# klepo/k-Wave-Fluid-CUDA

Measured on AMD Instinct MI355X. Metric: time-steps/sec on 256^3 heterogeneous grid; achieved HBM GB/s vs roofline, higher is better.
Workload: dtype f32; 1 GPU; 256^3 heterogeneous (c0,rho0,BonA,alpha_coeff arrays), power-law absorption + nonlinear, p0 source, p_raw+p_max on one xy plane (65536 points); fused_kernels=True, fft=hand-written fused FFT passes (kw_fused.hip), device=gfx950:sramecc+:xnack-

## Files before the change

### include/kwave_hip.h

```cpp
#ifndef KWAVE_HIP_H
#define KWAVE_HIP_H

#include <stddef.h>
#include <stdint.h>

#ifdef __cplusplus
extern "C" {
#endif

#define KW_API __attribute__((visibility("default")))

typedef struct kw_ctx kw_ctx;

typedef enum kw_status
{
  KW_OK            = 0,
  KW_ERR_INVALID   = 1,
  KW_ERR_HIP       = 2,
  KW_ERR_FFT       = 3,
  KW_ERR_ALLOC     = 4,
  KW_ERR_STATE     = 5,
  KW_ERR_NO_DEVICE = 6,
  KW_ERR_COMM      = 7
} kw_status;
// ... 39 lines not shown
  uint64_t l2_bytes;
} kw_device_info;

KW_API kw_status   kw_init(int device_id, kw_ctx** out_ctx);
KW_API kw_status   kw_destroy(kw_ctx* ctx);
KW_API const char* kw_last_error(void);
KW_API kw_status   kw_device_info_get(kw_ctx* ctx, kw_device_info* out);
KW_API kw_status   kw_set_stream(kw_ctx* ctx, void* hip_stream);
KW_API void*       kw_get_stream(kw_ctx* ctx);
KW_API kw_status   kw_sync(kw_ctx* ctx);
typedef struct kw_tuning
{
  uint32_t struct_bytes;
  int32_t  side_array;
  int32_t  tail_chunks;
  int32_t  split512;
  int32_t  slab_pipeline;
  int32_t  slab_chunks;
  int32_t  slab_batch;
  int32_t  p2p_blocks_per_peer;
  float    p2p_timeout_s;
  int32_t  plane_kernels;
  uint64_t offgrid_scratch_bytes;
} kw_tuning;
KW_API kw_status   kw_get_tuning(kw_ctx* ctx, kw_tuning* out);
KW_API kw_status   kw_set_tuning(kw_ctx* ctx, const kw_tuning* tuning);
typedef struct kw_graph kw_graph;
KW_API kw_status   kw_graph_begin(kw_ctx* ctx);
KW_API kw_status   kw_graph_end(kw_ctx* ctx, kw_graph** out);
KW_API kw_status   kw_graph_launch(kw_ctx* ctx, kw_graph* g);
KW_API kw_status   kw_graph_destroy(kw_ctx* ctx, kw_graph* g);
KW_API kw_status   kw_measure_copy_bandwidth(kw_ctx* ctx, size_t bytes, int reps, double* out_gbs);
KW_API kw_status   kw_event_create(kw_ctx* ctx, void** out_event);
KW_API kw_status   kw_event_record(kw_ctx* ctx, void* event);
KW_API kw_status   kw_event_synchronize(kw_ctx* ctx, void* event);
KW_API kw_status   kw_event_elapsed_ms(kw_ctx* ctx, void* start, void* stop, float* out_ms);
KW_API kw_status   kw_event_destroy(kw_ctx* ctx, void* event);

typedef struct kw_profile_entry
{
  char     name[64];
  uint64_t calls;
  double   total_ms;
} kw_profile_entry;
KW_API kw_status kw_profile_enable(kw_ctx* ctx, int on);
KW_API int       kw_profile_enabled(kw_ctx* ctx);
// ... 108 lines not shown
KW_API kw_status kw_comm_init_with(kw_ctx* ctx, const char* rccl_library, uint32_t nranks, uint32_t rank, const void* unique_id);
#define KW_COMM_P2P_BLOB_BYTES 1024
KW_API kw_status kw_comm_init_p2p(kw_ctx* ctx, uint32_t nranks, uint32_t rank);
KW_API kw_status kw_comm_p2p_export(kw_ctx* ctx, void* blob, size_t bytes);
KW_API kw_status kw_comm_p2p_connect(kw_ctx* ctx, const void* all_blobs);
KW_API kw_status kw_comm_p2p_emulate(kw_ctx* ctx, float link_gbs, float latency_us);
KW_API kw_status kw_comm_transport(kw_ctx* ctx, int* out_transport);
typedef int (*kw_exchange_fn)(void* user, void* send, void* recv, size_t bytes_per_peer);
KW_API kw_status kw_fused_set_slab(kw_ctx* ctx, uint32_t nranks, uint32_t rank, uint32_t nz_global,
                                   kw_exchange_fn exchange, void* user);
typedef int (*kw_exchange_start_fn)(void* user, void* send, void* recv, size_t bytes_per_peer, int slot);
typedef int (*kw_exchange_wait_fn)(void* user, int slot);
KW_API kw_status kw_fused_set_slab_async(kw_ctx* ctx, kw_exchange_start_fn start, kw_exchange_wait_fn wait);
typedef int (*kw_exchange_piece_fn)(void* user, void* send, void* recv, size_t stride_bytes, size_t offset_bytes, size_t bytes,
                                    int slot);
KW_API kw_status kw_fused_set_slab_pieces(kw_ctx* ctx, kw_exchange_piece_fn start, kw_exchange_wait_fn wait);
KW_API kw_status kw_fused_scratch_bytes(kw_ctx* ctx, size_t* out_bytes_per_array);
KW_API kw_status kw_fused_create_with_scratch(kw_ctx* ctx, void* const s[3], void* const t[3]);
KW_API kw_status kw_fused_supported(kw_ctx* ctx, int* out_supported);
KW_API kw_status kw_fused_create(kw_ctx* ctx);
KW_API kw_status kw_fused_destroy(kw_ctx* ctx);
KW_API kw_status kw_fused_reduced_elems(kw_ctx* ctx, size_t* out_floats);
KW_API kw_status kw_fused_import_reduced(kw_ctx* ctx, float* dst_padded, const float* src_reduced);
KW_API kw_status kw_fused_velocity(kw_ctx* ctx, const float* p, float* ux_sgx, float* uy_sgy, float* uz_sgz,
                                   const float* dt_rho0_sgx, const float* dt_rho0_sgy, const float* dt_rho0_sgz,
                                   const float* pml_x_sgx, const float* pml_y_sgy, const float* pml_z_sgz,
                                   const float* kappa_padded, const float* ddx_k_shift_pos,
                                   const float* ddy_k_shift_pos, const float* ddz_k_shift_pos, int chain_u_spectra);
#define KW_FUSED_CHAIN_U       1
#define KW_FUSED_P_IN_SCRATCH  2
#define KW_FUSED_U_IN_SCRATCH 1
#define KW_FUSED_CHAIN_TERMS  2
KW_API kw_status kw_fused_initial_velocity(kw_ctx* ctx, const float* p, float* ux_sgx, float* uy_sgy, float* uz_sgz,
                                           const float* dt_rho0_sgx, const float* dt_rho0_sgy,
                                           const float* dt_rho0_sgz, const float* kappa_padded,
                                           const float* ddx_k_shift_pos, const float* ddy_k_shift_pos,
                                           const float* ddz_k_shift_pos);
KW_API kw_status kw_fused_density(kw_ctx* ctx, int nonlinear, const float* ux_sgx, const float* uy_sgy,
                                  const float* uz_sgz, float* rho_x, float* rho_y, float* rho_z, const float* pml_x,
                                  const float* pml_y, const float* pml_z, const float* rho0,
                                  const float* kappa_padded, const float* ddx_k_shift_neg,
                                  const float* ddy_k_shift_neg, const float* ddz_k_shift_neg, float* duxdx,
                                  float* duydy, float* duzdz, int terms, const float* b_on_a, float* t0, float* t1,
                                  float* t2, int flags);
KW_API kw_status kw_fused_velocity_gradient(kw_ctx* ctx, const float* ux_sgx, const float* uy_sgy, const float* uz_sgz,
                                            float* duxdx, float* duydy, float* duzdz, const float* kappa_padded,
// ... 112 lines not shown
```

### k-wave-fluid-cuda_amd/capi.py

```python
from __future__ import annotations

import ctypes as C
import os
import re
from typing import Dict, Iterable, Optional

import numpy as np

PKG = os.path.dirname(os.path.abspath(__file__))
ROOT = os.path.dirname(PKG)
LIB_PATH = os.path.join(PKG, "lib", "libkwave_hip.so")
HEADER_PATH = os.path.join(ROOT, "include", "kwave_hip.h")

OP_NONE, OP_RMS, OP_MAX, OP_MIN = 0, 1, 2, 3
SRC_DIRICHLET, SRC_ADDITIVE_NO_CORRECTION, SRC_ADDITIVE = 0, 1, 2


class KWaveError(RuntimeError):
    """Non-zero kw_status; message = kw_last_error() (the reference throws std::runtime_error)."""


class Constants(C.Structure):
    _fields_ = [(n, C.c_uint32) for n in ("nx", "ny", "nz", "n_elements", "nx_complex", "ny_complex", "nz_complex",
                                          "n_elements_complex")] + \
# ... 102 lines not shown
    "kw_comm_init": [_P, C.c_uint32, C.c_uint32, _P],
    "kw_comm_destroy": [_P],
    "kw_comm_info": [_P, C.POINTER(C.c_uint32), C.POINTER(C.c_uint32), C.POINTER(C.c_uint64)],
    "kw_comm_unique_id_from": [C.c_char_p, _P, C.c_size_t],
    "kw_comm_init_with": [_P, C.c_char_p, C.c_uint32, C.c_uint32, _P],
    "kw_comm_init_p2p": [_P, C.c_uint32, C.c_uint32],
    "kw_comm_p2p_export": [_P, _P, C.c_size_t],
    "kw_comm_p2p_connect": [_P, _P],
    "kw_comm_p2p_emulate": [_P, C.c_float, C.c_float],
    "kw_comm_transport": [_P, C.POINTER(C.c_int)],
    "kw_get_tuning": [_P, _P],
    "kw_set_tuning": [_P, _P],
    "kw_fused_set_slab": [_P, C.c_uint32, C.c_uint32, C.c_uint32, _P, _P],
    "kw_fused_set_slab_async": [_P, _P, _P],
    "kw_fused_set_slab_pieces": [_P, _P, _P],
    "kw_fused_scratch_bytes": [_P, C.POINTER(C.c_size_t)],
    "kw_fused_create_with_scratch": [_P, _P, _P],
    "kw_fused_supported": [_P, C.POINTER(C.c_int)],
    "kw_fused_shift_velocity": [_P, C.c_int, _P, _P, _P],
    "kw_fused_create": [_P],
    "kw_fused_destroy": [_P],
    "kw_fused_reduced_elems": [_P, C.POINTER(C.c_size_t)],
    "kw_fused_import_reduced": [_P, _P, _P],
    "kw_fused_velocity": [_P] + [_P] * 14 + [C.c_int],
    "kw_fused_initial_velocity": [_P] + [_P] * 11,
    "kw_fused_density": [_P, C.c_int] + [_P] * 14 + [_P] * 3 + [C.c_int, _P, _P, _P, _P, C.c_int],
    "kw_fused_velocity_gradient": [_P] + [_P] * 10 + [C.c_int],
    "kw_fused_absorption_pressure": [_P] + [_P] * 9 + [C.c_int],
    "kw_fused_absorption_pressure_one": [_P] + [_P] * 6 + [C.c_int, C.c_int],
    "kw_fused_scale_source": [_P, _P, _P],
    "kw_fused_probe": [_P, C.c_int, _P],
    "kw_sample_index": [_P, C.c_int, _P, _P, _P, _U64],
    "kw_sample_index_multi": [_P, C.c_int, _P, _P, _P, _P, C.c_uint64],
    "kw_sample_cuboid": [_P, C.c_int, _P, _P, _P, _P, _P, _U64],
    "kw_sample_all": [_P, C.c_int, _P, _P, _U64],
    "kw_post_processing_rms": [_P, _P, C.c_float, _U64],
    "kw_sample_index_compress": [_P, _P, _P, _P, _P, _U64, C.c_uint32, _P, _P, C.c_uint32, C.c_uint32, C.c_int],
    "kw_sample_index_compress_40b": [_P, _P, _P, _P, _P, _U64, C.c_uint32, _P, _P, C.c_uint32, C.c_uint32, C.c_int, C.c_int, C.c_int],
    "kw_intensity_avg_c_accumulate_40b": [_P, _P, _P, _P, _U64, C.c_uint32, C.c_int, C.c_int],
    "kw_intensity_avg_c_accumulate": [_P, _P, _P, _P, _U64, C.c_uint32],
    "kw_time_shift_series": [_P, _P, _P, _U64, _U64],
    "kw_intensity_avg": [_P, _P, _P, _P, _U64, _U64],
    "kw_q_term_sum": [_P, _P, _P, _P, _P, _U64],
    "kw_divide": [_P, _P, C.c_float, _U64],
    "kw_element_source_row": [_P, _P, _P, _P, _P, C.c_uint32, C.c_uint32, _U64],
    "kw_sample_elements": [_P, _P, _P, _P, _P, C.c_uint32, _U64, _P, C.c_uint32, _P],
# ... 177 lines not shown
                                 C.byref(h)))
    try:
        n_el, nnz = _U64(), _U64()
        check(dev.L.kw_offgrid_size(dev.ctx, h, C.byref(n_el), C.byref(nnz)))
        ptr = np.empty(n_el.value + 1, dtype=np.uint64)
        index = np.empty(nnz.value, dtype=np.uint64)
        weight = np.empty(nnz.value, dtype=np.float32)
        check(dev.L.kw_offgrid_ptr(dev.ctx, h, ptr.ctypes.data))
        check(dev.L.kw_offgrid_entries(dev.ctx, h, index.ctypes.data, weight.ctypes.data))
    finally:
        dev.L.kw_offgrid_free(dev.ctx, h)
    return ptr, index, weight


COMM_ID_BYTES = 128
COMM_P2P_BLOB_BYTES = 1024
TRANSPORTS = {-1: "none", 0: "rccl", 1: "p2p (not connected)", 2: "p2p", 3: "p2p link model"}


class Tuning(C.Structure):
    _fields_ = [("struct_bytes", C.c_uint32), ("side_array", C.c_int32), ("tail_chunks", C.c_int32), ("split512", C.c_int32),
                ("slab_pipeline", C.c_int32), ("slab_chunks", C.c_int32), ("slab_batch", C.c_int32),
                ("p2p_blocks_per_peer", C.c_int32), ("p2p_timeout_s", C.c_float), ("plane_kernels", C.c_int32),
                ("offgrid_scratch_bytes", C.c_uint64)]


def default_tuning() -> Tuning:
    return Tuning(C.sizeof(Tuning), 1, 0, 1, 1, 1, -1, 4, 20.0, 1, 256 << 20)


def make_tuning(spec=None) -> Tuning:
    t = default_tuning()
    for src in (os.environ.get("KW_TUNING"), spec):
        if not src:
            continue
        items = src.items() if isinstance(src, dict) else (kv.split("=", 1) for kv in str(src).replace(" ", ",").split(",") if kv)
        for k, v in items:
            if k not in dict(Tuning._fields_) or k == "struct_bytes":
                raise KWaveError(f"unknown tuning parameter {k!r}")
            setattr(t, k, float(v) if k == "p2p_timeout_s" else int(v))
    return t


def comm_unique_id(rccl_library=None) -> bytes:
    buf = C.create_string_buffer(COMM_ID_BYTES)
    lib = rccl_library.encode() if rccl_library else None
    check(load().kw_comm_unique_id_from(lib, buf, COMM_ID_BYTES))
    return buf.raw


def comm_transport(ctx) -> str:
# ... 10 lines not shown
```

### k-wave-fluid-cuda_amd/csrc/kw_cw.hip

```cpp
#include "kw_fused.hip"

namespace {

template<int L> __global__ __launch_bounds__((Geo<L, nl_z(L)>::THREADS)) void k_zfused_pair(ZArgs a)
{
  using G = Geo<L, nl_z(L)>;
  constexpr int R1 = G::R1, R2 = G::R2;
  constexpr bool WA = (R2 == G::TPL) || ((G::NL * R2) % 64 == 0 && 64 % G::NL == 0);
  __shared__ float2 lds[G::LDSB];
  __shared__ float2 twl[G::TWN];
  load_twiddles<L>(twl, a.tw);
  const int       c     = threadIdx.x % G::NL;
  const int       j     = threadIdx.x / G::NL;
  const TileCoord tc    = tile_coord<G::NL>(a.nxc, a.P, a.side_off, gridDim.y, c);
  if (tc.dead) return;
  const uint32_t ky     = tc.pos;
  const bool     valid  = tc.valid;
  const uint32_t zstr   = a.ny * tc.pitch;
  const uint32_t base   = ky * tc.pitch + (tc.side ? 0u : tc.kx) + tc.off;
  const uint32_t basel  = ky * tc.pitch + tc.col + tc.off;
  constexpr int  OPV    = op_vec(R2);
  const uint32_t opbase = tc.side ? a.op_side_off + (((ky / NLMAX) * (R2 / OPV) * R1 + j) * NLMAX + ky % NLMAX) * OPV
                                  : (((ky * (a.Pop / NLMAX) + tc.col / NLMAX) * (R2 / OPV) * R1 + j) * NLMAX + tc.col % NLMAX) * OPV;
  const float2* __restrict__ in0 = a.in[0];
  const float2* __restrict__ in1 = a.in[1];

  float2 v[R1];
  if (ACTW(R2, j))
  {
    const uint32_t lb = (basel + static_cast<uint32_t>(j) * zstr) * static_cast<uint32_t>(sizeof(float2));
#pragma unroll
    for (int n1 = 0; n1 < R1; n1++) v[n1] = ld_uni<WA>(in0, static_cast<uint64_t>(n1 * R2) * zstr, lb);
  }
  float gr[R2], gi[R2];
  if (ACTW(R1, j))
  {
    load_op_run<R2, R1>(gr, a.op[0], opbase);
    load_op_run<R2, R1>(gi, a.op[1], opbase);
  }
  lds_barrier();

  if (ACTW(R2, j))
  {
    step_a<L, kFwd>(v, j, twl);
#pragma unroll
    for (int k1 = 0; k1 < R1; k1++) lds[k1 * G::SF + j * G::NL + c] = v[k1];
    uint32_t lb = basel + static_cast<uint32_t>(j) * zstr;
    asm volatile("" : "+v"(lb));
#pragma unroll
    for (int n1 = 0; n1 < R1; n1++)
      v[n1] = ld_uni<WA>(in1, static_cast<uint64_t>(n1 * R2) * zstr, lb * static_cast<uint32_t>(sizeof(float2)));
  }
  lds_barrier();
  float2 X[R2], Y[R2];
  if (ACTW(R1, j))
  {
#pragma unroll
    for (int n2 = 0; n2 < R2; n2++) X[n2] = lds[j * G::SF + n2 * G::NL + c];
    Dft<R2, kFwd>::run(X);
  }
  lds_barrier();
  if (ACTW(R2, j))
  {
    step_a<L, kFwd>(v, j, twl);
#pragma unroll
    for (int k1 = 0; k1 < R1; k1++) lds[k1 * G::SF + j * G::NL + c] = v[k1];
  }
  lds_barrier();
  if (ACTW(R1, j))
  {
#pragma unroll
    for (int n2 = 0; n2 < R2; n2++) Y[n2] = lds[j * G::SF + n2 * G::NL + c];
    Dft<R2, kFwd>::run(Y);
#pragma unroll
    for (int k2 = 0; k2 < R2; k2++)
    {
      const float2 x = X[k2], y = Y[k2];
      X[k2] = make_float2(gr[k2] * x.x - gi[k2] * y.x, gr[k2] * x.y - gi[k2] * y.y);
      Y[k2] = make_float2(gi[k2] * x.x + gr[k2] * y.x, gi[k2] * x.y + gr[k2] * y.y);
    }
  }

  float2 r[R1];
  inverse_from_regs<L, false, G::NL>(X, r, lds, c, j, twl);
  if (ACTW(R2, j) && valid)
  {
    float2* __restrict__ out = a.out[0];
    uint32_t ob = base + static_cast<uint32_t>(j) * zstr;
    asm volatile("" : "+v"(ob));
#pragma unroll
    for (int q2 = 0; q2 < R1; q2++) st_uni<WA>(out, static_cast<uint64_t>(R2 * q2) * zstr, ob * static_cast<uint32_t>(sizeof(float2)), r[q2]);
  }
  lds_barrier();
  inverse_from_regs<L, false, G::NL>(Y, r, lds, c, j, twl);
  if (ACTW(R2, j) && valid)
  {
// ... 331 lines not shown
      CV<V>::store(g.phase + s, vp);
    }
  }
}

}

namespace kwfused {

kw_status zfused_pair(kw_ctx* ctx, ZArgs a)
{
  const auto& f = ctx->fused;
  KW_PROF(ctx, "k_zfused_pair");
  a.tw          = f.tw[2];
  a.divider     = 1.0f;
  a.nxc         = f.nxm;
  a.side_off    = f.side_off;
  a.op_side_off = f.side_off;
  a.P           = f.P;
  a.Pop         = f.P;
  a.ny          = f.nyl;
  a.nz          = f.nz_global;
  a.narr        = 2;
  const uint32_t side_tile = (f.side_off != 0) ? 1u : 0u;
  if (f.nz_global == 512 && f.split512)
  {
    LAUNCH((k_zfused_pair_split<512>), dim3(f.P / NLMAX + side_tile, f.nyl, 1), dim3(Geo<256>::THREADS), a);
    return KW_OK;
  }
  const dim3 grid(z_tiles(f.P, f.nz_global) + side_tile, f.nyl, 1);
#define M(LEN) LAUNCH((k_zfused_pair<LEN>), grid, dim3((Geo<LEN, nl_z(LEN)>::THREADS)), a)
  KW_LEN_SWITCH(f.nz_global, M)
#undef M
  return KW_OK;
}

}

extern "C" {

kw_status kw_cw_operator(kw_ctx* ctx, float* g_re, float* g_im, double c0, double w, double T, double dkx, double dky,
                         double dkz)
{
  KW_CHECK_CONSTS(ctx);
  KW_PROF(ctx, "cw_operator");
  KW_REQUIRE(g_re && g_im);
// ... 75 lines not shown
```

### k-wave-fluid-cuda_amd/csrc/kw_fused.hip

```cpp
#ifndef KW_FUSED_HIP
#define KW_FUSED_HIP

#include "kw_fft_device.h"
#include "kw_internal.h"

#include <cmath>

using namespace kwfft;

#define KW_LONG_LINES 432

namespace kwfused {

struct RowAddr
{
  uint32_t magic, nyl, qstride, zmul;
  uint32_t estride;
  __device__ __forceinline__ uint32_t row(uint32_t z, uint32_t ky) const
  {
    const uint32_t q = (ky * magic) >> 20;
    return q * qstride + (ky - q * nyl) * estride + z * zmul;
  }
};

// ... 8 lines not shown
  uint32_t      z0;
  uint32_t      side_off;
  const float2* mul[3];
  RowAddr       ain, aout;
};

struct ZArgs
{
  const float2* in[3];
  float2*       out[3];
  const float*  op[2];
  const float2* dd[3];
  const float2* tw;
  float         divider;
  uint32_t      nxc, P, ny, nz;
  uint32_t      Pop;
  uint32_t      arr0;
  uint32_t      narr;
  uint32_t      ky0;
  uint32_t      lstride, bstride;
  uint32_t      side_off;
  uint32_t      op_side_off;
  uint32_t      axis_of[3];
};

struct XfwdArgs
{
  const float*  in[3];
  float2*       out[3];
  const float2* tw;
  uint32_t      nx, P;
  uint32_t      nrows, tile0;
  uint32_t      side_off;
};

struct XinvArgs
{
  const float2* in[3];
  const float2* tw;
  kw_constants  c;
  uint32_t      P;
  float*        out[3];
  const float*  m0[3];
  const float*  m1[3];
  float*        aux[3];
  float*        t[3];
// ... 40 lines not shown
kw_status xinv_density_stokes_long(int chain, kw_ctx* ctx, int ncomp, const XinvArgs& a, uint32_t tile0, uint32_t ntiles);
kw_status xinv_density_stokes_tail(int chain, kw_ctx* ctx, int ncomp, const XinvArgs& a, uint32_t tile0, uint32_t ntiles);
kw_status xinv_density_stokes_plane(int chain, kw_ctx* ctx, int ncomp, const XinvArgs& a, uint32_t plane0, uint32_t nplanes);
kw_status xinv_density_oneterm_short(int chain, kw_ctx* ctx, int ncomp, const XinvArgs& a, uint32_t tile0, uint32_t ntiles);
kw_status xinv_density_oneterm_long(int chain, kw_ctx* ctx, int ncomp, const XinvArgs& a, uint32_t tile0, uint32_t ntiles);
kw_status xinv_density_oneterm_tail(int chain, kw_ctx* ctx, int ncomp, const XinvArgs& a, uint32_t tile0, uint32_t ntiles);
kw_status xinv_density_oneterm_plane(int chain, kw_ctx* ctx, int ncomp, const XinvArgs& a, uint32_t plane0, uint32_t nplanes);
kw_status xinv_psum_one(int chain, kw_ctx* ctx, int ncomp, const XinvArgs& a, uint32_t tile0, uint32_t ntiles);
kw_status xinv_psum_one_tail(int chain, kw_ctx* ctx, int ncomp, const XinvArgs& a, uint32_t tile0, uint32_t ntiles);
kw_status xinv_psum_one_plane(int chain, kw_ctx* ctx, int ncomp, const XinvArgs& a, uint32_t plane0, uint32_t nplanes);
kw_status xinv_other(int epi, int chain, kw_ctx* ctx, int ncomp, const XinvArgs& a, uint32_t tile0, uint32_t ntiles);
kw_status xinv_other_tail(int epi, int chain, kw_ctx* ctx, int ncomp, const XinvArgs& a, uint32_t tile0, uint32_t ntiles);
kw_status xinv_density_plane(int chain, int terms, kw_ctx* ctx, int ncomp, const XinvArgs& a, uint32_t plane0, uint32_t nplanes);
kw_status xinv_other_plane(int epi, int chain, kw_ctx* ctx, int ncomp, const XinvArgs& a, uint32_t plane0, uint32_t nplanes);
kw_status zfused_pair(kw_ctx* ctx, ZArgs a);
kw_status yinv_angular(kw_ctx* ctx, AngArgs a);
kw_status probe_patterns(kw_ctx* ctx, int which, const float* op);

}
using namespace kwfused;

namespace {

constexpr int NLMAX = 16;
#ifdef KW_TUNE_NLX
constexpr int nl_x(int) { return KW_TUNE_NLX; }
#else
constexpr int nl_x(int L)
{
  switch (L)
  {
    case 100: case 108: case 140: case 160: case 168: case 196: case 200: case 224: case 288: case 336: case 384: case 392: return 8;
    case 280: case 300: case 320: case 432: case 480: case 500: case 600: return 10;
    case 180: case 216: case 240: case 252: case 324: case 360: case 400: return 12;
    case 896: return 16;
    default: return L >= 400 ? 8 : 16;
  }
}
#endif
constexpr bool has_partial_x_tiles(int L)
{
  switch (L)
  {
    case 672: case 700: case 720: case 756: case 784: case 800: case 840: case 864: case 900: case 960: return false;
    default: return true;
  }
// ... 133 lines not shown
  {
    const uint32_t p = blockIdx.y * NL + c;
    t.dead  = blockIdx.y * NL >= npos;
    t.kx    = nxc;
    t.col   = 0;
    t.valid = p < npos;
    t.pos   = min(p, npos - 1u);
    t.pitch = 1;
    t.off   = side_off;
    t.side  = true;
  }
  else
  {
    t.kx    = blockIdx.x * NL + c;
    t.col   = min(t.kx, nxc - 1u);
    t.valid = t.kx < nxc;
    t.pos   = blockIdx.y;
    t.pitch = P;
    t.off   = 0;
    t.dead  = false;
    t.side  = false;
  }
  return t;
}

template<int L> __device__ __forceinline__ void load_twiddles(float2* twl, const float2* __restrict__ tw)
{
  using G = Geo<L>;
  for (int e = threadIdx.x; e < G::R1 * G::R2; e += blockDim.x)
  {
    const int k = e / G::R2, n = e - k * G::R2;
    twl[k * G::TP + n] = tw[k * n];
  }
}

template<int L, int DIR> __device__ __forceinline__ void step_a(float2 (&v)[Fac<L>::R1], int n2, const float2* twl)
{
  Dft<Fac<L>::R1, DIR>::run(v);
#pragma unroll
  for (int k1 = 1; k1 < Fac<L>::R1; k1++) v[k1] = apply_tw<DIR>(v[k1], twl[k1 * Geo<L>::TP + n2]);
}


template<int L, int DIR, bool PIN, bool POUT>
__global__ __launch_bounds__(Geo<L>::THREADS) void k_ypass(PassArgs a)
{
// ... 109 lines not shown
    Dft<R1, kInv>::run(v);
  }
}

template<int L, int MODE> __global__ __launch_bounds__((Geo<L, nl_z(L)>::THREADS), big_line_waves(L)) void k_zfused(ZArgs a)
{
  using G = Geo<L, nl_z(L)>;
  constexpr int R1 = G::R1, R2 = G::R2;
  constexpr bool WA = (R2 == G::TPL) || ((G::NL * R2) % 64 == 0 && 64 % G::NL == 0);
  __shared__ float2 lds[G::LDSB];
  __shared__ float2 twl[G::TWN];
  load_twiddles<L>(twl, a.tw);
  const int      c      = threadIdx.x % G::NL;
  const int      j      = threadIdx.x / G::NL;
  const TileCoord tc    = tile_coord<G::NL>(a.nxc, a.P, (MODE == Z_SHIFT) ? 0u : a.side_off, gridDim.y, c);
  if (tc.dead) return;
  const uint32_t ky     = tc.pos;
  const bool     valid  = tc.valid;
  const uint32_t zstr   = (MODE == Z_SHIFT) ? a.lstride : a.ny * tc.pitch;
  const uint32_t bstr   = (MODE == Z_SHIFT) ? a.bstride : tc.pitch;
  const uint32_t kxl    = tc.kx < a.nxc ? tc.kx : (tc.side ? a.nxc : a.nxc - 1u);
  const uint32_t base   = ky * bstr + (tc.side ? 0u : tc.kx) + tc.off;
  const uint32_t basel  = ky * bstr + tc.col + tc.off;
  constexpr int  OPV    = op_vec(R2);
  const uint32_t opbase = tc.side ? a.op_side_off + (((ky / NLMAX) * (R2 / OPV) * R1 + j) * NLMAX + ky % NLMAX) * OPV
                                  : (((ky * (a.Pop / NLMAX) + tc.col / NLMAX) * (R2 / OPV) * R1 + j) * NLMAX + tc.col % NLMAX) * OPV;
  constexpr bool MULTI  = (MODE == Z_VGRAD || MODE == Z_ABSORB);
  const uint32_t arr0   = MULTI ? a.arr0 + blockIdx.z * a.narr : 0;
  const uint32_t narr   = MULTI ? a.narr : 1;
  constexpr int  NOUT   = (MODE == Z_PGRAD) ? 2 : 1;

  float2 v[R1];
  const float2* __restrict__ in0 = a.in[arr0];
  if (ACTW(R2, j))
  {
    const float2* __restrict__ in = in0;
    const uint32_t lb = (basel + static_cast<uint32_t>(j) * zstr) * static_cast<uint32_t>(sizeof(float2));
#pragma unroll
    for (int n1 = 0; n1 < R1; n1++)
      v[n1] = ld_uni<WA>(in, static_cast<uint64_t>(n1 * R2) * zstr, lb);
  }
  float kap[R2];
  if (MODE != Z_SHIFT && ACTW(R1, j))
  {
    load_op_run<R2, R1>(kap, a.op[(MODE == Z_ABSORB) ? arr0 : 0], opbase);
  }
  lds_barrier();

#pragma unroll 1
  for (uint32_t ia = 0; ia < narr; ia++)
  {
    const uint32_t arr = arr0 + ia;
    const float2* __restrict__ in_next = a.in[min(arr + 1u, arr0 + narr - 1u)];
    if (ACTW(R2, j))
    {
      step_a<L, kFwd>(v, j, twl);
#pragma unroll
      for (int k1 = 0; k1 < R1; k1++) lds[k1 * G::SF + j * G::NL + c] = v[k1];
    }
    if (MULTI && ia + 1 < narr && ACTW(R2, j))
    {
      const float2* __restrict__ in = in_next;
      uint32_t lb = basel + static_cast<uint32_t>(j) * zstr;
      asm volatile("" : "+v"(lb));
#pragma unroll
      for (int n1 = 0; n1 < R1; n1++)
        v[n1] = ld_uni<WA>(in, static_cast<uint64_t>(n1 * R2) * zstr, lb * static_cast<uint32_t>(sizeof(float2)));
    }
    lds_barrier();
    float2 X[R2];
    if (ACTW(R1, j))
    {
#pragma unroll
      for (int n2 = 0; n2 < R2; n2++) X[n2] = lds[j * G::SF + n2 * G::NL + c];
      Dft<R2, kFwd>::run(X);
      if (MODE == Z_SHIFT)
      {
#pragma unroll
        for (int k2 = 0; k2 < R2; k2++) X[k2] = cmulf(X[k2], a.dd[2][j + R1 * k2]);
      }
      else
      {
#pragma unroll
        for (int k2 = 0; k2 < R2; k2++)
        {
          float sc = kap[k2];
          if (MODE == Z_VGRAD || MODE == Z_SOURCE) sc *= a.divider;
          X[k2] = make_float2(X[k2].x * sc, X[k2].y * sc);
        }
      }
      if (MODE == Z_ABSORB && ia + 1 < narr)
      {
        uint32_t lb = opbase;
        asm volatile("" : "+v"(lb));
        load_op_run<R2, R1>(kap, a.op[arr + 1], lb);
      }
    }

#pragma unroll 1
    for (int o = 0; o < NOUT; o++)
    {
      float2 w[R2];
      if (ACTW(R1, j))
      {
        if (MODE == Z_PGRAD || MODE == Z_VGRAD)
        {
          const uint32_t axis = (MODE == Z_PGRAD) ? (o == 0 ? 3u : 2u) : a.axis_of[arr];
          if (axis == 3)
          {
#pragma unroll
            for (int k2 = 0; k2 < R2; k2++) w[k2] = X[k2];
          }
          else if (axis == 2)
          {
            uint32_t jz = j;
            asm volatile("" : "+v"(jz));
#pragma unroll
            for (int k2 = 0; k2 < R2; k2++) w[k2] = cmulf(X[k2], a.dd[2][jz + R1 * k2]);
// ... 1087 lines not shown
```

### k-wave-fluid-cuda_amd/csrc/kw_fused_main.hip

```cpp
#include "kw_fused.hip"

#include <cmath>
#include <cstdlib>
#include <cstring>
#include <vector>

namespace {

__global__ __launch_bounds__(256) void k_import_reduced(float* __restrict__ dst, const float* __restrict__ src, uint32_t nxc,
                                                        uint32_t nxm, uint32_t P, uint32_t nyl, uint32_t nzg, uint32_t r1,
                                                        uint32_t vec, uint32_t split)
{
  __shared__ float tile[NLMAX * 1024];
  const uint32_t nt = P / NLMAX, t = blockIdx.x % nt, ky = blockIdx.x / nt;
  const uint32_t n = NLMAX * nzg;
  for (uint32_t i = threadIdx.x; i < n; i += blockDim.x)
  {
    const uint32_t kz = i / NLMAX, kx = t * NLMAX + i % NLMAX;
    tile[i] = (kx < nxm) ? src[(static_cast<size_t>(kz) * nyl + ky) * nxc + kx] : 0.f;
  }
  __syncthreads();
  float* __restrict__ out = dst + static_cast<size_t>(blockIdx.x) * n;
  for (uint32_t p = threadIdx.x; p < n; p += blockDim.x)
  {
    uint32_t r = p;
    const uint32_t v  = r % vec; r /= vec;
    const uint32_t c  = r % NLMAX; r /= NLMAX;
    const uint32_t j  = r % r1;
    const uint32_t q  = r / r1;
    const uint32_t ri = q * vec + v;
    const uint32_t kz = split ? 2u * j + (ri & 1u) + 2u * r1 * (ri >> 1) : j + r1 * ri;
    out[p] = tile[kz * NLMAX + c];
  }
}
__global__ void k_import_reduced_side(float* __restrict__ dst, const float* __restrict__ src, uint32_t nxc, uint32_t nyl,
                                      uint32_t nzg, size_t total, uint32_t r1, uint32_t vec, uint32_t split)
{
  const uint32_t nq = nzg / (r1 * vec);
  for (size_t e = static_cast<size_t>(blockIdx.x) * blockDim.x + threadIdx.x; e < total;
       e += static_cast<size_t>(gridDim.x) * blockDim.x)
  {
    size_t         r  = e;
    const uint32_t r4 = static_cast<uint32_t>(r % vec); r /= vec;
    const uint32_t c  = static_cast<uint32_t>(r % NLMAX); r /= NLMAX;
    const uint32_t j  = static_cast<uint32_t>(r % r1); r /= r1;
    const uint32_t q  = static_cast<uint32_t>(r % nq); r /= nq;
    const uint32_t ky = static_cast<uint32_t>(r) * NLMAX + c;
    const uint32_t ri = q * vec + r4;
    const uint32_t kz = split ? 2u * j + (ri & 1u) + 2u * r1 * (ri >> 1) : j + r1 * ri;
    dst[e] = (ky < nyl) ? src[(static_cast<size_t>(kz) * nyl + ky) * nxc + (nxc - 1u)] : 0.f;
  }
}

bool supported_len(uint32_t n)
{
#define X(LEN) if (n == LEN) return true;
  KW_FUSED_LENGTHS(X)
#undef X
  return false;
}

#define KW_FUSED_READY(ctx)                                                                                            \
  do {                                                                                                                 \
    KW_CHECK_CONSTS(ctx);                                                                                              \
    if (!(ctx)->fused.ready) { kw_set_error("%s: kw_fused_create has not been called", __func__); return KW_ERR_STATE; } \
  } while (0)

#define KW_TRY(call) KW_TRY_STATUS(call)

kw_status launch_xfwd(kw_ctx* ctx, int narr, const float* const* in, float2* const* out, uint32_t nzc = 0)
{
  const kw_constants& c = ctx->c;
  static const char* const names[3] = { "k_xfwd[1]", "k_xfwd[2]", "k_xfwd[3]" };
  KW_PROF(ctx, names[narr - 1]);
// ... 81 lines not shown
  const kw_constants& c = ctx->c;
  const auto& f = ctx->fused;
  static const char* const names[4][3] = { { "k_zfused_pgrad", "k_zfused_pgrad", "k_zfused_pgrad" },
                                           { "k_zfused_vgrad[1]", "k_zfused_vgrad[2]", "k_zfused_vgrad[3]" },
                                           { "k_zfused_absorb[1]", "k_zfused_absorb[2]", "k_zfused_absorb[3]" },
                                           { "k_zfused_source", "k_zfused_source", "k_zfused_source" } };
  KW_PROF(ctx, names[MODE][narr - 1]);
  if (f.pipelined)
  {
    for (int i = 0; i < 3; i++)
      for (int j = 0; j < 3; j++)
      {
        if (a.in[i] == f.s[j]) a.in[i] = f.r[j];
        if (a.out[i] == f.s[j]) a.out[i] = f.r[j];
      }
  }
  a.tw      = f.tw[2];
  a.divider = c.fft_divider;
  a.nxc     = f.nxm;
  a.axis_of[0] = 0; a.axis_of[1] = f.two_d ? 2u : 1u; a.axis_of[2] = 2;
  if (f.two_d) a.dd[2] = a.dd[1];
  a.side_off    = f.side_off;
  a.op_side_off = f.side_off;
  const uint32_t side_tile = (f.side_off != 0) ? 1u : 0u;
  a.P       = f.slab ? f.PX : f.P;
  a.Pop     = f.P;
  a.ny      = f.nyl;
  a.nz      = f.nz_global;
  a.ky0     = f.rank * f.nyl;
  a.narr    = narr;
  if (f.nz_global == 512 && f.split512)
  {
    LAUNCH((k_zfused_split<512, MODE>), dim3(f.P / NLMAX + side_tile, f.nyl, narr), dim3(Geo<256>::THREADS), a);
    return KW_OK;
  }
  uint32_t split = 1;
  if ((MODE == Z_VGRAD || MODE == Z_ABSORB) && narr > 1 &&
      (z_tiles(f.P, f.nz_global) + side_tile) * f.nyl < 2u * static_cast<uint32_t>(ctx->cu_count))
  {
    split  = static_cast<uint32_t>(narr);
    a.narr = 1;
  }
  const dim3 grid(z_tiles(f.P, f.nz_global) + side_tile, f.nyl, split);
#define M(LEN) LAUNCH((k_zfused<LEN, MODE>), grid, dim3((Geo<LEN, nl_z(LEN)>::THREADS)), a)
  KW_LEN_SWITCH(f.nz_global, M)
#undef M
// ... 502 lines not shown
    uint32_t nch = static_cast<uint32_t>(tn.slab_chunks > 0 ? tn.slab_chunks : 1);
    if (nch > KW_XCHUNKS_MAX) nch = KW_XCHUNKS_MAX;
    while (nch > 1 && (c.nz % nch != 0 || (c.nz / nch * c.ny) % (2 * nl_x(c.nx)) != 0)) nch--;
    f.xchunks = f.pipelined ? nch : 1u;
    const size_t per_peer = static_cast<size_t>(c.nz) * f.nyl * c.nx_complex * sizeof(float2);
    f.xbatch = f.pipelined && ((tn.slab_batch >= 0) ? (tn.slab_batch == 1) : (per_peer < (4u << 20)));
    if (f.xbatch) f.xchunks = 1u;
  }
  KW_TRY(alloc_scratch(ctx, s, t));
  const uint32_t lens[3] = { c.nx, c.ny, f.nz_global };
  for (int i = 0; i < 3; i++)
  {
    std::vector<float2> tw(lens[i]);
    for (uint32_t m = 0; m < lens[i]; m++)
    {
      const double ph = -2.0 * M_PI * static_cast<double>(m) / static_cast<double>(lens[i]);
      tw[m]           = make_float2(static_cast<float>(std::cos(ph)), static_cast<float>(std::sin(ph)));
    }
    KW_HIP(hipMalloc(reinterpret_cast<void**>(&f.tw[i]), lens[i] * sizeof(float2)));
    KW_HIP(hipMemcpyAsync(f.tw[i], tw.data(), lens[i] * sizeof(float2), hipMemcpyHostToDevice, ctx->stream));
    KW_HIP(hipStreamSynchronize(ctx->stream));
  }
  f.split512 = (ctx->tuning.split512 != 0);
  f.plane = (ctx->tuning.plane_kernels != 0) && !f.slab && !f.two_d && c.nx == c.ny && plane_len(static_cast<int>(c.nx)) &&
            supported_len(c.nx);
  if (f.plane)
  {
    const size_t elems = static_cast<size_t>(f.Palloc) * c.ny * c.nz;
    KW_HIP(hipMalloc(reinterpret_cast<void**>(&f.s4), elems * sizeof(float2)));
    KW_HIP(hipMemsetAsync(f.s4, 0, elems * sizeof(float2), ctx->stream));
  }
  f.ready = true;
  return KW_OK;
}

}

extern "C" {

kw_status kw_fused_set_slab(kw_ctx* ctx, uint32_t nranks, uint32_t rank, uint32_t nz_global, kw_exchange_fn fn, void* user)
{
  KW_CHECK_CTX(ctx);
  KW_REQUIRE(nranks >= 1 && rank < nranks);
  if (ctx->fused.ready) { kw_set_error("kw_fused_set_slab: must be called before kw_fused_create"); return KW_ERR_STATE; }
  uint32_t comm_ranks = 0, comm_rank = 0;
  KW_TRY(kw_comm_info(ctx, &comm_ranks, &comm_rank, nullptr));
// ... 104 lines not shown
  return KW_OK;
}

kw_status kw_fused_import_reduced(kw_ctx* ctx, float* dst_padded, const float* src)
{
  KW_FUSED_READY(ctx);
  KW_REQUIRE(dst_padded && src);
  const kw_constants& c = ctx->c;
  const bool split = (ctx->fused.nz_global == 512 && ctx->fused.split512);
  uint32_t r1 = Fac<256>::R1, r2 = Fac<256>::R2;
  if (!split)
    switch (ctx->fused.nz_global)
    {
#define X(LEN) case LEN: r1 = Fac<LEN>::R1; r2 = Fac<LEN>::R2; break;
      KW_FUSED_LENGTHS(X)
#undef X
      default: kw_set_error("kw_fused_import_reduced: unsupported length %u", ctx->fused.nz_global); return KW_ERR_INVALID;
    }
  const uint32_t vec = static_cast<uint32_t>(op_vec(static_cast<int>(split ? 2 * r2 : r2)));
  const auto& f = ctx->fused;
  const size_t main_total = static_cast<size_t>(c.ny) * c.nz * f.P;
  KW_REQUIRE(f.nz_global <= 1024);
  KW_HIP(hipMemsetAsync(dst_padded, 0, static_cast<size_t>(f.Palloc) * c.ny * c.nz * sizeof(float), ctx->stream));
  LAUNCH(k_import_reduced, dim3(f.nyl * (f.P / NLMAX)), dim3(256), dst_padded, src, c.nx_complex, f.nxm, f.P, f.nyl, f.nz_global,
         r1, vec, split ? 1u : 0u);
  if (f.side_off != 0)
  {
    const size_t side_total = static_cast<size_t>((f.nyl + NLMAX - 1) / NLMAX) * NLMAX * f.nz_global;
    LAUNCH(k_import_reduced_side, dim3(ctx->cu_count * 2), dim3(256), dst_padded + main_total, src, c.nx_complex, f.nyl,
           f.nz_global, side_total, r1, vec, split ? 1u : 0u);
  }
  return KW_OK;
}

kw_status kw_fused_velocity(kw_ctx* ctx, const float* p, float* ux, float* uy, float* uz, const float* dtx,
                            const float* dty, const float* dtz, const float* pmlx, const float* pmly, const float* pmlz,
                            const float* kappa_padded, const float* ddx, const float* ddy, const float* ddz,
                            int chain_u_spectra)
{
  KW_FUSED_READY(ctx);
  KW_PROF(ctx, "fused_velocity");
  KW_REQUIRE(p && ux && uy && uz && pmlx && pmly && pmlz && kappa_padded && ddx && ddy && ddz);
  KW_REQUIRE((dtx == nullptr) == (dty == nullptr) && (dtx == nullptr) == (dtz == nullptr));
  float2** S = ctx->fused.s;
  const float* in1[1] = { p };
  const bool p_in_scratch = (chain_u_spectra & KW_FUSED_P_IN_SCRATCH) != 0;
  chain_u_spectra &= KW_FUSED_CHAIN_U;
  KW_TRY(forward_xy(ctx, 1, p_in_scratch ? nullptr : in1));
  ZArgs z{};
  z.in[0] = S[0];
  for (int i = 0; i < 3; i++) z.out[i] = S[i];
  z.op[0] = kappa_padded;
  z.dd[0] = (const float2*)ddx; z.dd[1] = (const float2*)ddy; z.dd[2] = (const float2*)ddz;
  KW_TRY(launch_zfused<Z_PGRAD>(ctx, 1, z));
// ... 475 lines not shown
```

### k-wave-fluid-cuda_amd/csrc/kw_internal.h

```cpp
#ifndef KW_INTERNAL_H
#define KW_INTERNAL_H

#include <hip/hip_runtime.h>
#include <rocfft/rocfft.h>

#include <cstdarg>
#include <cstdio>
#include <cstring>
#include <vector>

#include "kwave_hip.h"

struct kw_fft_plan
{
  rocfft_plan           plan  = nullptr;
  rocfft_execution_info info  = nullptr;
  size_t                work  = 0;
};

struct kw_comm_state;
inline kw_tuning kw_tuning_defaults()
{
  kw_tuning t{};
  t.struct_bytes        = static_cast<uint32_t>(sizeof(kw_tuning));
  t.side_array          = 1;
  t.tail_chunks         = 0;
  t.split512            = 1;
  t.slab_pipeline       = 1;
  t.slab_chunks         = 1;
  t.slab_batch          = -1;
  t.p2p_blocks_per_peer = 4;
  t.p2p_timeout_s       = 20.f;
  t.plane_kernels       = 1;
  t.offgrid_scratch_bytes = 256ull << 20;
  return t;
}
#define KW_COMM_SLOTS 32
#define KW_XCHUNKS_MAX 4

struct kw_ctx
{
  int          device      = 0;
  hipStream_t  own_stream  = nullptr;
  hipStream_t  stream      = nullptr;
  hipStream_t  copy_stream = nullptr;
  hipEvent_t   copy_fence  = nullptr;
  bool         have_consts = false;
  kw_constants c{};
  int          cu_count    = 256;
  bool         fft_setup   = false;
  kw_fft_plan  r2c_3d, c2r_3d;
  kw_fft_plan  r2c_1d[3], c2r_1d[3];
  void*        fft_work       = nullptr;
  size_t       fft_work_bytes = 0;
  struct fused_plan
  {
    bool     ready = false;
// ... 6 lines not shown
    uint32_t P     = 0;
    uint32_t PX    = 0;
    float2*  s[3]  = {nullptr, nullptr, nullptr};
    float2*  s4    = nullptr;
    float2*  tw[3] = {nullptr, nullptr, nullptr};
    uint32_t nranks = 1, rank = 0, nz_global = 0, nyl = 0;
    bool     slab   = false;
    float2*  t[3]  = {nullptr, nullptr, nullptr};
    bool     owns_scratch = true;
    kw_exchange_fn exchange = nullptr;
    void*          exchange_user = nullptr;
    kw_exchange_start_fn exchange_start = nullptr;
    kw_exchange_wait_fn  exchange_wait  = nullptr;
    kw_exchange_piece_fn exchange_piece = nullptr;
    bool     two_d = false;
    bool     pipelined = false;
    uint32_t xchunks   = 1;
    float2*  r[3]      = {nullptr, nullptr, nullptr};
    int      fwd_ahead = 0;
    bool     xbatch    = false;
    int8_t   xslot[2][3][KW_XCHUNKS_MAX] = {};
    bool     slot_waited[KW_COMM_SLOTS] = {};
    int8_t   slot_pieces[KW_COMM_SLOTS] = {};
  } fused;
  kw_comm_state* comm = nullptr;
  kw_tuning      tuning = kw_tuning_defaults();
  struct prof_rec { const char* name; hipEvent_t e0, e1; };
  bool                  profiling = false;
  std::vector<prof_rec> prof;
};

struct kw_prof_scope
{
  kw_ctx* ctx;
  size_t  idx;
  bool    on;
  kw_prof_scope(kw_ctx* c, const char* name) : ctx(c), idx(0), on(c && c->profiling)
  {
    if (!on) return;
    kw_ctx::prof_rec r{name, nullptr, nullptr};
    if (hipEventCreate(&r.e0) != hipSuccess || hipEventCreate(&r.e1) != hipSuccess) { on = false; return; }
    (void)hipEventRecord(r.e0, ctx->stream);
    idx = ctx->prof.size();
    ctx->prof.push_back(r);
  }
  ~kw_prof_scope()
// ... 73 lines not shown
```

Before: 1127 time-steps/s.

## Fold mirror-symmetric spectral operators to halve operator storage and loads

When an imported k-space operator (kappa, absorption terms) is symmetric under ky→ny-ky and kz→nz-kz, it is stored only for the half-range of ky and about half the z runs. Kernels then index the mirrored row or run and reverse the per-thread register run. A device check decides at import time whether the operator is symmetric, and only those buffers are marked folded. The aim is to cut HBM traffic for operator reads in the z-pass kernels, at the cost of extra index math, a host sync at import, and a pointer-identity registry that could go stale.

```diff
diff --git a/include/kwave_hip.h b/include/kwave_hip.h
--- a/include/kwave_hip.h
+++ b/include/kwave_hip.h
@@ -85,6 +85,7 @@
   float    p2p_timeout_s;
   int32_t  plane_kernels;
   uint64_t offgrid_scratch_bytes;
+  int32_t  fold_operators;
 } kw_tuning;
 KW_API kw_status   kw_get_tuning(kw_ctx* ctx, kw_tuning* out);
 KW_API kw_status   kw_set_tuning(kw_ctx* ctx, const kw_tuning* tuning);
@@ -239,6 +240,7 @@
 KW_API kw_status kw_fused_destroy(kw_ctx* ctx);
 KW_API kw_status kw_fused_reduced_elems(kw_ctx* ctx, size_t* out_floats);
 KW_API kw_status kw_fused_import_reduced(kw_ctx* ctx, float* dst_padded, const float* src_reduced);
+KW_API kw_status kw_fused_operator_folded(kw_ctx* ctx, const float* padded, int* out);
 KW_API kw_status kw_fused_velocity(kw_ctx* ctx, const float* p, float* ux_sgx, float* uy_sgy, float* uz_sgz,
                                    const float* dt_rho0_sgx, const float* dt_rho0_sgy, const float* dt_rho0_sgz,
                                    const float* pml_x_sgx, const float* pml_y_sgy, const float* pml_z_sgz,
diff --git a/k-wave-fluid-cuda_amd/capi.py b/k-wave-fluid-cuda_amd/capi.py
--- a/k-wave-fluid-cuda_amd/capi.py
+++ b/k-wave-fluid-cuda_amd/capi.py
@@ -148,6 +148,7 @@
     "kw_fused_destroy": [_P],
     "kw_fused_reduced_elems": [_P, C.POINTER(C.c_size_t)],
     "kw_fused_import_reduced": [_P, _P, _P],
+    "kw_fused_operator_folded": [_P, _P, C.POINTER(C.c_int)],
     "kw_fused_velocity": [_P] + [_P] * 14 + [C.c_int],
     "kw_fused_initial_velocity": [_P] + [_P] * 11,
     "kw_fused_density": [_P, C.c_int] + [_P] * 14 + [_P] * 3 + [C.c_int, _P, _P, _P, _P, C.c_int],
@@ -371,11 +372,11 @@
     _fields_ = [("struct_bytes", C.c_uint32), ("side_array", C.c_int32), ("tail_chunks", C.c_int32), ("split512", C.c_int32),
                 ("slab_pipeline", C.c_int32), ("slab_chunks", C.c_int32), ("slab_batch", C.c_int32),
                 ("p2p_blocks_per_peer", C.c_int32), ("p2p_timeout_s", C.c_float), ("plane_kernels", C.c_int32),
-                ("offgrid_scratch_bytes", C.c_uint64)]
+                ("offgrid_scratch_bytes", C.c_uint64), ("fold_operators", C.c_int32)]
 
 
 def default_tuning() -> Tuning:
-    return Tuning(C.sizeof(Tuning), 1, 0, 1, 1, 1, -1, 4, 20.0, 1, 256 << 20)
+    return Tuning(C.sizeof(Tuning), 1, 0, 1, 1, 1, -1, 4, 20.0, 1, 256 << 20, 1)
 
 
 def make_tuning(spec=None) -> Tuning:
diff --git a/k-wave-fluid-cuda_amd/csrc/kw_cw.hip b/k-wave-fluid-cuda_amd/csrc/kw_cw.hip
--- a/k-wave-fluid-cuda_amd/csrc/kw_cw.hip
+++ b/k-wave-fluid-cuda_amd/csrc/kw_cw.hip
@@ -19,9 +19,7 @@
   const uint32_t zstr   = a.ny * tc.pitch;
   const uint32_t base   = ky * tc.pitch + (tc.side ? 0u : tc.kx) + tc.off;
   const uint32_t basel  = ky * tc.pitch + tc.col + tc.off;
-  constexpr int  OPV    = op_vec(R2);
-  const uint32_t opbase = tc.side ? a.op_side_off + (((ky / NLMAX) * (R2 / OPV) * R1 + j) * NLMAX + ky % NLMAX) * OPV
-                                  : (((ky * (a.Pop / NLMAX) + tc.col / NLMAX) * (R2 / OPV) * R1 + j) * NLMAX + tc.col % NLMAX) * OPV;
+  const bool     revj   = fold_reversed<G>(j);
   const float2* __restrict__ in0 = a.in[0];
   const float2* __restrict__ in1 = a.in[1];
 
@@ -33,10 +31,11 @@
     for (int n1 = 0; n1 < R1; n1++) v[n1] = ld_uni<WA>(in0, static_cast<uint64_t>(n1 * R2) * zstr, lb);
   }
   float gr[R2], gi[R2];
+  const bool fr = !tc.side && (a.op_fold & 1u) != 0, fi = !tc.side && (a.op_fold & 2u) != 0;
   if (ACTW(R1, j))
   {
-    load_op_run<R2, R1>(gr, a.op[0], opbase);
-    load_op_run<R2, R1>(gi, a.op[1], opbase);
+    load_op<G>(gr, a.op[0], op_run_base<G>(a, tc, ky, j, fr, fr && revj), fr);
+    load_op<G>(gi, a.op[1], op_run_base<G>(a, tc, ky, j, fi, fi && revj), fi);
   }
   lds_barrier();
 
@@ -72,6 +71,16 @@
 #pragma unroll
     for (int n2 = 0; n2 < R2; n2++) Y[n2] = lds[j * G::SF + n2 * G::NL + c];
     Dft<R2, kFwd>::run(Y);
+    if (fr && revj)
+    {
+#pragma unroll
+      for (int k2 = 0; k2 < R2 / 2; k2++) { const float t = gr[k2]; gr[k2] = gr[R2 - 1 - k2]; gr[R2 - 1 - k2] = t; }
+    }
+    if (fi && revj)
+    {
+#pragma unroll
+      for (int k2 = 0; k2 < R2 / 2; k2++) { const float t = gi[k2]; gi[k2] = gi[R2 - 1 - k2]; gi[R2 - 1 - k2] = t; }
+    }
 #pragma unroll
     for (int k2 = 0; k2 < R2; k2++)
     {
@@ -449,6 +458,7 @@
   a.ny          = f.nyl;
   a.nz          = f.nz_global;
   a.narr        = 2;
+  a.op_fold     = op_fold_bits(ctx, a);
   const uint32_t side_tile = (f.side_off != 0) ? 1u : 0u;
   if (f.nz_global == 512 && f.split512)
   {
diff --git a/k-wave-fluid-cuda_amd/csrc/kw_fused.hip b/k-wave-fluid-cuda_amd/csrc/kw_fused.hip
--- a/k-wave-fluid-cuda_amd/csrc/kw_fused.hip
+++ b/k-wave-fluid-cuda_amd/csrc/kw_fused.hip
@@ -54,6 +54,7 @@
   uint32_t      side_off;
   uint32_t      op_side_off;
   uint32_t      axis_of[3];
+  uint32_t      op_fold;
 };
 
 struct XfwdArgs
@@ -140,6 +141,15 @@
 
 namespace {
 
+inline uint32_t op_fold_bits(const kw_ctx* ctx, const ZArgs& a)
+{
+  uint32_t bits = 0;
+  for (int i = 0; i < 2; i++)
+    for (const void* p : ctx->fused.folded)
+      if (a.op[i] != nullptr && p == a.op[i]) bits |= 1u << i;
+  return bits;
+}
+
 constexpr int NLMAX = 16;
 #ifdef KW_TUNE_NLX
 constexpr int nl_x(int) { return KW_TUNE_NLX; }
@@ -319,6 +329,44 @@
     t.side  = false;
   }
   return t;
+}
+
+constexpr int fold_runs(int r1) { return r1 / 2 + 1; }
+template<class G> struct FoldGeo
+{
+  static constexpr int  RH      = (G::R1 + 1) / 2;
+  static constexpr bool UNIFORM = (G::NL * RH) % 64 == 0 && 64 % G::NL == 0;
+};
+template<class G> __device__ __forceinline__ bool fold_reversed(int j)
+{
+  return FoldGeo<G>::UNIFORM ? __builtin_amdgcn_readfirstlane(j) >= FoldGeo<G>::RH : j >= FoldGeo<G>::RH;
+}
+template<class G>
+__device__ __forceinline__ uint32_t op_run_base(const ZArgs& a, const TileCoord& tc, uint32_t ky, int j, bool fold, bool rev)
+{
+  constexpr int R1 = G::R1, R2 = G::R2, OPV = op_vec(R2);
+  if (tc.side) return a.op_side_off + (((ky / NLMAX) * (R2 / OPV) * R1 + j) * NLMAX + ky % NLMAX) * OPV;
+  const uint32_t tile = (fold ? min(ky, a.ny - ky) : ky) * (a.Pop / NLMAX) + tc.col / NLMAX;
+  const uint32_t run  = fold ? tile * static_cast<uint32_t>((R2 / OPV) * fold_runs(R1)) + static_cast<uint32_t>(rev ? R1 - j : j)
+                             : tile * static_cast<uint32_t>((R2 / OPV) * R1) + static_cast<uint32_t>(j);
+  return (run * NLMAX + tc.col % NLMAX) * OPV;
+}
+template<class G>
+__device__ __forceinline__ void load_op(float (&dst)[G::R2], const float* __restrict__ op, uint32_t base, bool fold)
+{
+  if (fold) load_op_run<G::R2, fold_runs(G::R1)>(dst, op, base);
+  else load_op_run<G::R2, G::R1>(dst, op, base);
+}
+template<int RUN, bool DIV, bool REV>
+__device__ __forceinline__ void scale_by_run(float2 (&X)[RUN], const float (&run)[RUN], float divider)
+{
+#pragma unroll
+  for (int k2 = 0; k2 < RUN; k2++)
+  {
+    float sc = run[REV ? RUN - 1 - k2 : k2];
+    if (DIV) sc *= divider;
+    X[k2] = make_float2(X[k2].x * sc, X[k2].y * sc);
+  }
 }
 
 template<int L> __device__ __forceinline__ void load_twiddles(float2* twl, const float2* __restrict__ tw)
@@ -474,9 +522,7 @@
   const uint32_t kxl    = tc.kx < a.nxc ? tc.kx : (tc.side ? a.nxc : a.nxc - 1u);
   const uint32_t base   = ky * bstr + (tc.side ? 0u : tc.kx) + tc.off;
   const uint32_t basel  = ky * bstr + tc.col + tc.off;
-  constexpr int  OPV    = op_vec(R2);
-  const uint32_t opbase = tc.side ? a.op_side_off + (((ky / NLMAX) * (R2 / OPV) * R1 + j) * NLMAX + ky % NLMAX) * OPV
-                                  : (((ky * (a.Pop / NLMAX) + tc.col / NLMAX) * (R2 / OPV) * R1 + j) * NLMAX + tc.col % NLMAX) * OPV;
+  const bool     revj   = fold_reversed<G>(j);
   constexpr bool MULTI  = (MODE == Z_VGRAD || MODE == Z_ABSORB);
   const uint32_t arr0   = MULTI ? a.arr0 + blockIdx.z * a.narr : 0;
   const uint32_t narr   = MULTI ? a.narr : 1;
@@ -493,9 +539,13 @@
       v[n1] = ld_uni<WA>(in, static_cast<uint64_t>(n1 * R2) * zstr, lb);
   }
   float kap[R2];
+  bool  rev = false;
   if (MODE != Z_SHIFT && ACTW(R1, j))
   {
-    load_op_run<R2, R1>(kap, a.op[(MODE == Z_ABSORB) ? arr0 : 0], opbase);
+    const uint32_t oi   = (MODE == Z_ABSORB) ? arr0 : 0;
+    const bool     fold = !tc.side && ((a.op_fold >> oi) & 1u) != 0;
+    rev = fold && revj;
+    load_op<G>(kap, a.op[oi], op_run_base<G>(a, tc, ky, j, fold, rev), fold);
   }
   lds_barrier();
 
@@ -531,21 +581,15 @@
 #pragma unroll
         for (int k2 = 0; k2 < R2; k2++) X[k2] = cmulf(X[k2], a.dd[2][j + R1 * k2]);
       }
-      else
-      {
-#pragma unroll
-        for (int k2 = 0; k2 < R2; k2++)
-        {
-          float sc = kap[k2];
-          if (MODE == Z_VGRAD || MODE == Z_SOURCE) sc *= a.divider;
-          X[k2] = make_float2(X[k2].x * sc, X[k2].y * sc);
-        }
-      }
+      else if (rev) scale_by_run<R2, (MODE == Z_VGRAD || MODE == Z_SOURCE), true>(X, kap, a.divider);
+      else scale_by_run<R2, (MODE == Z_VGRAD || MODE == Z_SOURCE), false>(X, kap, a.divider);
       if (MODE == Z_ABSORB && ia + 1 < narr)
       {
-        uint32_t lb = opbase;
+        const bool fold = !tc.side && ((a.op_fold >> (arr + 1u)) & 1u) != 0;
+        rev = fold && revj;
+        uint32_t lb = op_run_base<G>(a, tc, ky, j, fold, rev);
         asm volatile("" : "+v"(lb));
-        load_op_run<R2, R1>(kap, a.op[arr + 1], lb);
+        load_op<G>(kap, a.op[arr + 1], lb, fold);
       }
     }
 
diff --git a/k-wave-fluid-cuda_amd/csrc/kw_fused_main.hip b/k-wave-fluid-cuda_amd/csrc/kw_fused_main.hip
--- a/k-wave-fluid-cuda_amd/csrc/kw_fused_main.hip
+++ b/k-wave-fluid-cuda_amd/csrc/kw_fused_main.hip
@@ -9,25 +9,25 @@
 
 __global__ __launch_bounds__(256) void k_import_reduced(float* __restrict__ dst, const float* __restrict__ src, uint32_t nxc,
                                                         uint32_t nxm, uint32_t P, uint32_t nyl, uint32_t nzg, uint32_t r1,
-                                                        uint32_t vec, uint32_t split)
+                                                        uint32_t vec, uint32_t split, uint32_t jh)
 {
   __shared__ float tile[NLMAX * 1024];
   const uint32_t nt = P / NLMAX, t = blockIdx.x % nt, ky = blockIdx.x / nt;
-  const uint32_t n = NLMAX * nzg;
+  const uint32_t n = NLMAX * nzg, nout = NLMAX * (nzg / r1) * jh;
   for (uint32_t i = threadIdx.x; i < n; i += blockDim.x)
   {
     const uint32_t kz = i / NLMAX, kx = t * NLMAX + i % NLMAX;
     tile[i] = (kx < nxm) ? src[(static_cast<size_t>(kz) * nyl + ky) * nxc + kx] : 0.f;
   }
   __syncthreads();
-  float* __restrict__ out = dst + static_cast<size_t>(blockIdx.x) * n;
-  for (uint32_t p = threadIdx.x; p < n; p += blockDim.x)
+  float* __restrict__ out = dst + static_cast<size_t>(blockIdx.x) * nout;
+  for (uint32_t p = threadIdx.x; p < nout; p += blockDim.x)
   {
     uint32_t r = p;
     const uint32_t v  = r % vec; r /= vec;
     const uint32_t c  = r % NLMAX; r /= NLMAX;
-    const uint32_t j  = r % r1;
-    const uint32_t q  = r / r1;
+    const uint32_t j  = r % jh;
+    const uint32_t q  = r / jh;
     const uint32_t ri = q * vec + v;
     const uint32_t kz = split ? 2u * j + (ri & 1u) + 2u * r1 * (ri >> 1) : j + r1 * ri;
     out[p] = tile[kz * NLMAX + c];
@@ -50,6 +50,24 @@
     const uint32_t kz = split ? 2u * j + (ri & 1u) + 2u * r1 * (ri >> 1) : j + r1 * ri;
     dst[e] = (ky < nyl) ? src[(static_cast<size_t>(kz) * nyl + ky) * nxc + (nxc - 1u)] : 0.f;
   }
+}
+
+__global__ __launch_bounds__(256) void k_check_mirror(uint32_t* __restrict__ flag, const uint32_t* __restrict__ src, uint32_t nxc,
+                                                      uint32_t nxm, uint32_t ny, uint32_t nz)
+{
+  const size_t total = static_cast<size_t>(nz) * ny * nxm;
+  bool differs = false;
+  for (size_t e = static_cast<size_t>(blockIdx.x) * blockDim.x + threadIdx.x; e < total;
+       e += static_cast<size_t>(gridDim.x) * blockDim.x)
+  {
+    const uint32_t kx = static_cast<uint32_t>(e % nxm);
+    const uint32_t ky = static_cast<uint32_t>((e / nxm) % ny), kz = static_cast<uint32_t>(e / (static_cast<size_t>(nxm) * ny));
+    const uint32_t my = ky ? ny - ky : 0u, mz = kz ? nz - kz : 0u;
+    const uint32_t v  = src[(static_cast<size_t>(kz) * ny + ky) * nxc + kx];
+    differs = differs || v != src[(static_cast<size_t>(kz) * ny + my) * nxc + kx] ||
+              v != src[(static_cast<size_t>(mz) * ny + ky) * nxc + kx];
+  }
+  if (differs) *flag = 1u;
 }
 
 bool supported_len(uint32_t n)
@@ -177,6 +195,7 @@
   if (f.two_d) a.dd[2] = a.dd[1];
   a.side_off    = f.side_off;
   a.op_side_off = f.side_off;
+  a.op_fold     = op_fold_bits(ctx, a);
   const uint32_t side_tile = (f.side_off != 0) ? 1u : 0u;
   a.P       = f.slab ? f.PX : f.P;
   a.Pop     = f.P;
@@ -725,6 +744,7 @@
     KW_HIP(hipStreamSynchronize(ctx->stream));
   }
   f.split512 = (ctx->tuning.split512 != 0);
+  f.fold_ops = (ctx->tuning.fold_operators != 0) && !f.slab && !f.two_d && f.nranks == 1;
   f.plane = (ctx->tuning.plane_kernels != 0) && !f.slab && !f.two_d && c.nx == c.ny && plane_len(static_cast<int>(c.nx)) &&
             supported_len(c.nx);
   if (f.plane)
@@ -875,14 +895,41 @@
   const size_t main_total = static_cast<size_t>(c.ny) * c.nz * f.P;
   KW_REQUIRE(f.nz_global <= 1024);
   KW_HIP(hipMemsetAsync(dst_padded, 0, static_cast<size_t>(f.Palloc) * c.ny * c.nz * sizeof(float), ctx->stream));
-  LAUNCH(k_import_reduced, dim3(f.nyl * (f.P / NLMAX)), dim3(256), dst_padded, src, c.nx_complex, f.nxm, f.P, f.nyl, f.nz_global,
-         r1, vec, split ? 1u : 0u);
+  auto& folded = ctx->fused.folded;
+  for (size_t i = 0; i < folded.size();)
+    if (folded[i] == dst_padded) folded.erase(folded.begin() + static_cast<ptrdiff_t>(i)); else i++;
+  bool fold = f.fold_ops && !split;
+  if (fold)
+  {
+    uint32_t differs = 0;
+    LAUNCH(k_check_mirror, dim3(ctx->cu_count * 4), dim3(256), reinterpret_cast<uint32_t*>(dst_padded),
+           reinterpret_cast<const uint32_t*>(src), c.nx_complex, f.nxm, c.ny, c.nz);
+    KW_HIP(hipMemcpyAsync(&differs, dst_padded, sizeof(differs), hipMemcpyDeviceToHost, ctx->stream));
+    KW_HIP(hipStreamSynchronize(ctx->stream));
+    if (differs != 0) KW_HIP(hipMemsetAsync(dst_padded, 0, sizeof(differs), ctx->stream));
+    fold = (differs == 0);
+  }
+  if (fold) folded.push_back(dst_padded);
+  const uint32_t rows = fold ? c.ny / 2u + 1u : f.nyl, jh = fold ? static_cast<uint32_t>(fold_runs(static_cast<int>(r1))) : r1;
+  LAUNCH(k_import_reduced, dim3(rows * (f.P / NLMAX)), dim3(256), dst_padded, src, c.nx_complex, f.nxm, f.P, f.nyl, f.nz_global,
+         r1, vec, split ? 1u : 0u, jh);
   if (f.side_off != 0)
   {
     const size_t side_total = static_cast<size_t>((f.nyl + NLMAX - 1) / NLMAX) * NLMAX * f.nz_global;
     LAUNCH(k_import_reduced_side, dim3(ctx->cu_count * 2), dim3(256), dst_padded + main_total, src, c.nx_complex, f.nyl,
            f.nz_global, side_total, r1, vec, split ? 1u : 0u);
   }
+  return KW_OK;
+}
+
+kw_status kw_fused_operator_folded(kw_ctx* ctx, const float* padded, int* out)
+{
+  KW_FUSED_READY(ctx);
+  KW_REQUIRE(out != nullptr);
+  *out = 0;
+  if (padded == nullptr) *out = static_cast<int>(ctx->fused.folded.size());
+  for (const void* p : ctx->fused.folded)
+    if (p == padded) *out = 1;
   return KW_OK;
 }
 
diff --git a/k-wave-fluid-cuda_amd/csrc/kw_internal.h b/k-wave-fluid-cuda_amd/csrc/kw_internal.h
--- a/k-wave-fluid-cuda_amd/csrc/kw_internal.h
+++ b/k-wave-fluid-cuda_amd/csrc/kw_internal.h
@@ -33,6 +33,7 @@
   t.p2p_timeout_s       = 20.f;
   t.plane_kernels       = 1;
   t.offgrid_scratch_bytes = 256ull << 20;
+  t.fold_operators      = 1;
   return t;
 }
 #define KW_COMM_SLOTS 32
@@ -85,6 +86,8 @@
     int8_t   xslot[2][3][KW_XCHUNKS_MAX] = {};
     bool     slot_waited[KW_COMM_SLOTS] = {};
     int8_t   slot_pieces[KW_COMM_SLOTS] = {};
+    bool     fold_ops = false;
+    std::vector<const void*> folded;
   } fused;
   kw_comm_state* comm = nullptr;
   kw_tuning      tuning = kw_tuning_defaults();
```

Result: no change. 1139 time-steps/s (median of 6 runs) (+1.1%).
